# mcgill-cpslab/all-pairs-similarity

Hardware: AMD Instinct MI355X
Metric: scored candidate pairs/sec + achieved HBM GB/s, N=1M d=100k nnz=100, 1/2/4/8 GPU (higher is better)
Workload: dtype u16+f32

## Files before the change

### all-pairs-similarity_amd/csrc/apss_even.hpp

```cpp
#pragma once
#include "apss_kernels.hpp"

namespace apss {

template <int BLOCK, int U, int LONGCAP, bool SHARD, bool SIGNED, bool ACC8, bool MERGE>
__device__ __forceinline__ void probe_even_body(const ProbeArgs &a) {
  constexpr int NW = BLOCK / kWave;
  static_assert(NW == 8 || NW == 16, "8 or 16 waves");
  constexpr int NS = NW - 1;
  constexpr bool SLOT2 = BLOCK <= 512;
  constexpr uint32_t ABITS = ACC8 ? 8u : 16u;
  constexpr bool WIDE = ACC8 && BLOCK > 512;
  constexpr int CH = 16, LPC = CH / 2, GPW = kWave / LPC, WIN = GPW * U;
  constexpr int SLOTS = 2 * WIN < 48 ? 2 * WIN : (WIN > 48 ? WIN : 48);
  static_assert(SLOTS >= WIN, "the register window reads the first WIN slots of a strip");
  constexpr int GS = BLOCK > 512 ? SLOTS / GPW : ((SLOTS / GPW) + 1) & ~1;
  constexpr int SSZ = GPW * GS;
  static_assert(GPW == 8 && SLOTS % GPW == 0, "slot <-> (step, group) by shifts");
  constexpr int kLongLen = kLongLenW;
  constexpr int CBMAX = WIDE ? 131072 : (BLOCK <= 512 && !ACC8 ? 32768 : 65536);
  constexpr int APW = 32 / (int)ABITS;
  constexpr bool LEAN = !SIGNED;
  static_assert(1 + (NW - 1) * 2 * U < (1 << (ACC8 ? 8 : 16)), "the spare words' low accumulators must not wrap within a round");
  __shared__ __attribute__((aligned(16))) uint32_t acc[CBMAX / APW + kWave];
  __shared__ __attribute__((aligned(16))) uint2 strips[3 * NS * SSZ + kWave];
  __shared__ uint2 longs[3 * LONGCAP];
  __shared__ float long_w[3 * LONGCAP];
  __shared__ uint2 facts[4];
  __shared__ unsigned long long stat[4];
  unsigned char *const smem_raw = reinterpret_cast<unsigned char *>(acc);
  uint32_t *const facts_w = reinterpret_cast<uint32_t *>(facts);

  const int tid = threadIdx.x;
  const int wv = __builtin_amdgcn_readfirstlane(tid / kWave), ln = tid % kWave;
  const int cb = a.cb;
  const int F = a.flat_waves;
  const int A = NW - F;
  const int CAP = A * SLOTS;
  const uint32_t A8 = (uint32_t)A * (uint32_t)GPW;
  const float rcpA8 = 1.0f / (float)A8;
  const uint32_t magicA8 = 0xffffffffu / A8 + 1u;
  const int LOGG = a.flat_group_log2, G = 1 << LOGG;
  const uint32_t sub = (uint32_t)ln & (uint32_t)(G - 1);
  const int tile = a.tile0 + blockIdx.x / a.n_chunks;
  const int chunk = blockIdx.x % a.n_chunks;
  static_assert(!MERGE || SHARD, "merged rounds: term shards only");
  const int mlaunch = MERGE ? a.merge_log2 : 0;
  const int c0 = chunk * a.q_chunk;
  const int row_lo = c0 << mlaunch, row_hi = MERGE ? min(a.nq_rows, (c0 + a.q_chunk) << mlaunch) : 0;
  const bool own_tile = mlaunch != 0 && a.q_slot_base >= 0 && (a.q_slot_base + row_lo) / cb <= tile && tile <= (a.q_slot_base + row_hi - 1) / cb;
  const int mlog = own_tile ? 0 : mlaunch;
  const int v0 = row_lo >> mlog;
  const int v1 = own_tile ? row_hi : min(a.nq, c0 + a.q_chunk);
  const int nv = own_tile ? a.nq_rows : a.nq;
  const int qtile = row_lo / cb;
  if (a.tri && tile > qtile) return;
  const int64_t tile_row0 = (int64_t)tile * cb;
  const int unmerged_mark = own_tile ? kUnmergedBit : 0;
  const uint32_t lo = (uint32_t)(ln % LPC);
  const float cxs = a.cx_scale;

  const int64_t qbase = a.q_rowptr[MERGE ? min(v0 << mlog, a.nq_rows) : v0], qend = a.q_rowptr[MERGE ? min(v1 << mlog, a.nq_rows) : v1];
  const int64_t pbase = a.tile_post_base[tile], pend = a.tile_post_base[tile + 1];
  const __amdgpu_buffer_rsrc_t rs_qi =
      __builtin_amdgcn_make_buffer_rsrc((void *)(a.q_idx + qbase), 0, (int)((qend - qbase) * 4), 0x00020000);
  const __amdgpu_buffer_rsrc_t rs_qv =
      __builtin_amdgcn_make_buffer_rsrc((void *)(a.q_val + qbase), 0, (int)((qend - qbase) * 4), 0x00020000);
  const __amdgpu_buffer_rsrc_t rs_tp = __builtin_amdgcn_make_buffer_rsrc(
      (void *)(a.tile_seg + (int64_t)tile * a.seg_stride), 0, (int)(a.seg_stride * 8), 0x00020000);
  const __amdgpu_buffer_rsrc_t rs_po =
      __builtin_amdgcn_make_buffer_rsrc((void *)(a.post_c + pbase), 0, (int)((pend - pbase) * 4), 0x00020000);
  constexpr uint32_t kOob = 0xfffffff0u;
  constexpr uint32_t kStale = 0x80000000u, kSwept = 0x40000000u;
  constexpr uint32_t kRare = 0x80000000u;
  constexpr uint32_t kCountMask = 0xffffu;
  constexpr int kFirstSkippable = BLOCK > 512 || !SHARD ? U - 1 : 0;

  for (int i = tid * 4; i < cb / APW; i += BLOCK * 4) *reinterpret_cast<uint4 *>(acc + i) = make_uint4(0u, 0u, 0u, 0u);
  if (tid < kWave) acc[CBMAX / APW + tid] = 1u;
  if (LEAN) {
    for (int i = tid; i < 3 * NS * SSZ; i += BLOCK) strips[i].x = kStale;
  }
  if (tid < 8) facts_w[tid] = 0;
  unsigned long long my_visits = 0;
  uint32_t my_cands = 0;
  uint32_t n_seen = 0;

  struct RowExt { int qb; int nnz; };
  struct TermW { uint32_t term; float w, qs; bool valid; };
  struct Seg { uint32_t s, len; float w; };
  struct WaveWork {
    uint32_t info;
    uint32_t flags;
    apss_u32x2 pc[U];
    float wq[U];
  };
  const int32_t *const rowptr_lo = reinterpret_cast<const int32_t *>(a.q_rowptr);
  const int qbase_lo = (int)(uint32_t)qbase;
  auto load_R = [&](int v) {
    RowExt r;
    const int row_a = min(v, nv - 1) << mlog, row_b = MERGE ? min(row_a + (1 << mlog), a.nq_rows) : row_a + 1;
    r.qb = rowptr_lo[2 * row_a];
    r.nnz = rowptr_lo[2 * row_b];
    return r;
  };
  auto load_I = [&](const RowExt &r, const int fi, const int v) {
    TermW t;
    const int kterm = ((fi * kWave) >> LOGG) + (ln >> LOGG);
    const int nnz = v < v1 ? r.nnz - r.qb : 0;
    t.valid = kterm < nnz;
    const uint32_t off = t.valid ? (uint32_t)(r.qb - qbase_lo + kterm) * 4u : kOob;
// ... 336 lines not shown
            *reinterpret_cast<unsigned short *>(smem_raw + (w0.pc[u].x & 0xffffu)) = 0;
            *reinterpret_cast<unsigned short *>(smem_raw + (w0.pc[u].y & 0xffffu)) = 0;
          } else {
            acc16w[w0.pc[u].x & 0xffffu] = 0;
            acc16w[w0.pc[u].y & 0xffffu] = 0;
          }
        }
      }
      __syncthreads();
    };
    int r0 = 0;
    for (int v = v0; v < v1; v += 2) {
      round(wfa, wfb, v, r0);
      r0 = r0 == 2 ? 0 : r0 + 1;
      if (v + 1 >= v1) break;
      round(wfb, wfa, v + 1, r0);
      r0 = r0 == 2 ? 0 : r0 + 1;
    }
  }
  __syncthreads();
  if (tid < 3) stat[tid] = 0;
  __syncthreads();
  atomicAdd(&stat[0], my_visits);
  atomicAdd(&stat[1], (unsigned long long)(my_cands - n_seen));
  __syncthreads();
  if (tid == 0) {
    const unsigned long long twice = a.tri && tile < qtile ? 2ull : 1ull;
    atomicAdd(&a.counters[kCtrVisits], stat[0] * twice);
    atomicAdd(&a.counters[kCtrCands], stat[1] * twice);
    atomicAdd(&a.counters[kCtrDevVisits], stat[0]);
  }
}

template <int BLOCK, int U, int LONGCAP, bool SHARD, bool SIGNED, bool ACC8>
__global__ __launch_bounds__(BLOCK, BLOCK <= 512 ? 2 * BLOCK / 256 : BLOCK / 256) void k_probe_even(const ProbeArgs a) {
  probe_even_body<BLOCK, U, LONGCAP, SHARD, SIGNED, ACC8, false>(a);
}

template <int U, bool ACC8>
__global__ __launch_bounds__(512, 4) void k_probe_even_merged(const ProbeArgs a) {
  probe_even_body<512, U, 128, true, false, ACC8, true>(a);
}

}
```

### all-pairs-similarity_amd/csrc/apss_hip.hip

```cpp
#include <hip/hip_runtime.h>

#include <algorithm>
#include <cmath>
#include <cstdio>
#include <cstdlib>
#include <cstring>
#include <new>
#include <string>
#include <vector>

#include "../../include/apss.h"
#include "apss_kernels.hpp"
#include "apss_head.hpp"
#include "apss_even.hpp"
#include "apss_topk.hpp"
#include "apss_window.hpp"

using namespace apss;

namespace {

thread_local std::string g_create_error;

template <class T>
struct DevBuf {
  T *p = nullptr;
  size_t cap = 0;
};

struct DebugCfg {
  bool build_lds = false;
  bool build_atomic = false;
  bool build_stream = false;
  bool build_runs = false;
  int run_range = 0;
  int run_lanes = 0;
  int run_sub = -1;
  bool build_trace = false;
  bool chunk8 = false;
  bool shard_exact = false;
  bool diag = false;
  bool force_general = false;
  bool exact_accum = false;
  bool big_u5 = false;
  int cx_tile = 0;
  int window = 0;
  int chunks = 0;
  int tiles_per_launch = 0;
  bool no_tail = false;
  bool no_acc8 = false;
  int flat_group = -1;
  int pad_lds = 0;
  bool longpf = false;
  bool even_wide = false;
  bool no_even = false;
  int seg_align = 0;
  bool bank_order = false;
  int fold_w = 0;
  bool no_sym = false;
  int mix = 0;
  bool no_chain = false;
  bool no_append = false;
  bool no_bucket = false;
  int bucket_range = 0;
  int res_cap = 0;
  bool head_bf16 = false;
  int merge = -1;
  bool no_merge_prune = false;
  int merge_u = 0;
  int merge_single = 0;
  bool no_fused_ingest = false;
};

DebugCfg parse_debug_env() {
  DebugCfg d;
  const char *e = getenv("APSS_DEBUG");
  if (!e) return d;
  std::string str(e);
  size_t pos = 0;
  while (pos <= str.size()) {
    const size_t end = std::min(str.find(',', pos), str.size());
    const std::string tok = str.substr(pos, end - pos);
    pos = end + 1;
    const size_t eq = tok.find('=');
    const std::string key = tok.substr(0, eq);
    const int val = eq == std::string::npos ? 1 : atoi(tok.c_str() + eq + 1);
    if (key == "build_lds") d.build_lds = val != 0;
    else if (key == "build_atomic") d.build_atomic = val != 0;
    else if (key == "build_stream") d.build_stream = val != 0;
    else if (key == "build_runs") d.build_runs = val != 0;
    else if (key == "run_range") d.run_range = val;
    else if (key == "run_lanes") d.run_lanes = val;
    else if (key == "run_sub") d.run_sub = val;
    else if (key == "build_trace") d.build_trace = val != 0;
    else if (key == "chunk8") d.chunk8 = val != 0;
    else if (key == "shard_exact") d.shard_exact = val != 0;
    else if (key == "diag") d.diag = val != 0;
    else if (key == "force_general") d.force_general = val != 0;
    else if (key == "exact_accum") d.exact_accum = val != 0;
    else if (key == "big_u5") d.big_u5 = val != 0;
    else if (key == "cx_tile") d.cx_tile = val;
    else if (key == "window") d.window = val;
    else if (key == "chunks") d.chunks = val;
    else if (key == "tiles_per_launch") d.tiles_per_launch = val;
    else if (key == "no_tail") d.no_tail = val != 0;
    else if (key == "no_acc8") d.no_acc8 = val != 0;
    else if (key == "no_even") d.no_even = val != 0;
    else if (key == "even_wide") d.even_wide = val != 0;
    else if (key == "longpf") d.longpf = val != 0;
    else if (key == "pad_lds") d.pad_lds = (int)val;
    else if (key == "flat_group") d.flat_group = (int)val;
    else if (key == "seg_align") d.seg_align = val;
    else if (key == "bank_order") d.bank_order = val != 0;
    else if (key == "fold_w") d.fold_w = val;
    else if (key == "mix") d.mix = val;
    else if (key == "no_sym") d.no_sym = val != 0;
    else if (key == "no_chain") d.no_chain = val != 0;
    else if (key == "no_append") d.no_append = val != 0;
    else if (key == "head_bf16") d.head_bf16 = val != 0;
    else if (key == "res_cap") d.res_cap = val;
    else if (key == "no_bucket") d.no_bucket = val != 0;
    else if (key == "bucket_range") d.bucket_range = val;
    else if (key == "merge") d.merge = (int)val;
    else if (key == "merge_u") d.merge_u = (int)val;
    else if (key == "no_merge_prune") d.no_merge_prune = val != 0;
    else if (key == "merge_single") d.merge_single = (int)val;
    else if (key == "no_fused_ingest") d.no_fused_ingest = val != 0;
    else if (key == "relayout_fail") {}
    else if (!key.empty()) fprintf(stderr, "[apss] unknown APSS_DEBUG token '%s' ignored\n", key.c_str());
  }
  return d;
}

}

struct apss_handle {
  apss_config cfg{};
  DebugCfg dbgcfg;
  int dev = 0;
  hipStream_t own_stream = nullptr;
  hipStream_t stream = nullptr;
  hipEvent_t ev0 = nullptr, ev1 = nullptr;
  std::string err;
  bool sharded = false;
  bool nonneg = true;
  bool q_nonneg = true;
  bool no_acc8 = false;
  uint32_t downgrades = 0;
  int64_t store_max_nnz = 0, q_max_nnz = 0;
  float store_max_norm2 = 0.f, q_max_norm2 = 0.f;
  int64_t store_nonempty = 0;
  int64_t last_batch_nonempty = 0;
  int32_t cb = 16384;
  bool stored_rows = false;

  int64_t n_rows = 0, nnz = 0;
  int64_t idx_rows = 0;
  DevBuf<int64_t> rowptr, ext;
  DevBuf<int32_t> idx;
  DevBuf<uint32_t> erow;
// ... 83 lines not shown
    DevBuf<uint32_t> erow;
    int64_t rows = 0, nnz = 0, max_nnz = 0, nonempty = 0, last_nonempty = 0;
  };
  TailView tv, qtv;
  DevBuf<int64_t> tv_cnt, tv_off;
  DevBuf<unsigned int> tv_sum;
  DevBuf<uint16_t> W, q_W;
  bool head_i8 = false;
  float head_s = 0.f;
  DevBuf<unsigned int> head_ovf;
  DevBuf<uint32_t> df;
  DevBuf<unsigned long long> dedup_tab, head_ctr;
  DevBuf<int32_t> uq_q, uq_c;
  DevBuf<float> uq_s;
  int64_t head_nonempty = 0, last_batch_head_nonempty = 0;
  double head_sample_frac = 0.0;
  hipEvent_t ev2 = nullptr, ev3 = nullptr;
  int32_t top_k = 0;
  TopkWork topk;
  apss_topk_info tk{};
  int64_t top_k_window = 0;
  DevBuf<unsigned int> win_df;
  DevBuf<int32_t> win_b;
  DevBuf<int32_t> win_q, win_c;
  DevBuf<float> win_s;
  std::vector<int64_t> win_cuts;
  apss_topk_window_info tw{};
  int64_t win_nonempty = -1, win_head_nonempty = -1;
  bool tile_cut = false, cut_ran = false;
  int64_t cut_uncut = 0, cut_rounds = 0;
  DevBuf<uint32_t> row_pairs;
  apss_topk_tile_cut_info tci{};
  int64_t probe_reruns = 0;
  apss_stats st{};
  size_t bytes_reserved = 0;
};

namespace {

#define HIPCHK(h, expr)                                                                              \
  do {                                                                                               \
    hipError_t e_ = (expr);                                                                          \
    if (e_ != hipSuccess) {                                                                          \
      (h)->err = std::string(#expr) + ": " + hipGetErrorString(e_);                                  \
      return e_ == hipErrorOutOfMemory ? APSS_E_NOMEM : APSS_E_DEVICE;                               \
    }                                                                                                \
  } while (0)

#define APSS_TRY(expr)          \
  do {                          \
    int32_t rc_ = (expr);       \
    if (rc_ != APSS_OK) return rc_; \
  } while (0)

int32_t fail(apss_handle *h, int32_t rc, const std::string &msg) {
  h->err = msg;
  return rc;
}

template <class T>
int32_t ensure(apss_handle *h, DevBuf<T> &b, size_t n, size_t keep = 0, bool exact = false) {
  if (n <= b.cap && b.p) return APSS_OK;
  size_t ncap = exact ? n : std::max(n, b.cap + b.cap / 2);
  ncap = std::max<size_t>(ncap, 64);
  T *np = nullptr;
  HIPCHK(h, hipMalloc((void **)&np, ncap * sizeof(T)));
// ... 1159 lines not shown
  X(1024, 3, false, false, false)      \
  X(1024, 7, false, false, true)       \
  X(1024, 6, false, false, true)       \
  X(1024, 5, false, false, true)       \
  X(1024, 3, false, false, true)
#define APSS_EVEN_MERGE_VARIANTS(X) \
  X(7, false) X(6, false) X(5, false) X(4, false) X(3, false) X(2, false) \
  X(7, true) X(6, true) X(5, true) X(4, true) X(3, true) X(2, true)

bool cx_variant_exists(const CxVariant &v) {
  if (v.even && v.merge) {
#define X(U, A8) \
    if (v.block == 512 && v.u == U && v.shard && !v.sgn && v.acc8 == A8) return v.chunk == 16 && !v.vrows && !v.longpf;
    APSS_EVEN_MERGE_VARIANTS(X)
#undef X
    return false;
  }
  if (v.even) {
#define X(B, U, SH, SG, A8) \
    if (v.block == B && v.u == U && v.shard == SH && v.sgn == SG && v.acc8 == A8) return v.chunk == 16 && !v.vrows && !v.longpf;
    APSS_EVEN_VARIANTS(X)
#undef X
    return false;
  }
#define X(B, U, SH, CH, VR, SG, LP, A8)                                                                                 \
  if (v.block == B && v.u == U && v.shard == SH && v.chunk == CH && v.vrows == VR && v.sgn == SG && v.longpf == LP &&   \
      v.acc8 == A8)                                                                                                     \
    return true;
  APSS_CX_VARIANTS(X)
#undef X
  return false;
}

int32_t launch_cx(apss_handle *h, const CxVariant &v, const ProbeArgs &a) {
  const dim3 grid((unsigned)((int64_t)a.n_tiles * a.n_chunks));
  if (v.even && v.merge) {
#define X(U, A8)                                                                                                           \
    if (v.block == 512 && v.u == U && v.acc8 == A8) {                                                                      \
      hipLaunchKernelGGL((k_probe_even_merged<U, A8>), grid, dim3(512), (size_t)h->dbgcfg.pad_lds, h->stream, a);           \
      HIPCHK(h, hipGetLastError());                                                                                        \
      return APSS_OK;                                                                                                      \
    }
    APSS_EVEN_MERGE_VARIANTS(X)
#undef X
    return fail(h, APSS_E_UNSUPPORTED, "no filter kernel for this combination of options");
  }
  if (v.even) {
#define X(B, U, SH, SG, A8)                                                                                                \
    if (v.block == B && v.u == U && v.shard == SH && v.sgn == SG && v.acc8 == A8) {                                        \
      hipLaunchKernelGGL((k_probe_even<B, U, (B <= 512 ? 128 : 256), SH, SG, A8>), grid, dim3(B),                          \
                         (size_t)h->dbgcfg.pad_lds, h->stream, a);                                                                                 \
      HIPCHK(h, hipGetLastError());                                                                                        \
      return APSS_OK;                                                                                                      \
    }
    APSS_EVEN_VARIANTS(X)
#undef X
    return fail(h, APSS_E_UNSUPPORTED, "no filter kernel for this combination of options");
  }
#define X(B, U, SH, CH, VR, SG, LP, A8)                                                                                    \
  if (v.block == B && v.u == U && v.shard == SH && v.chunk == CH && v.vrows == VR && v.sgn == SG && v.longpf == LP &&      \
      v.acc8 == A8) {                                                                                                      \
    hipLaunchKernelGGL((k_probe_coarse<B, U, (B <= 512 ? 128 : 256), (B <= 512 ? 512 : 1024), SH, CH, VR, SG, LP, A8>), grid, dim3(B), \
                       0, h->stream, a);                                                                                   \
    HIPCHK(h, hipGetLastError());                                                                                          \
    return APSS_OK;                                                                                                        \
  }
  APSS_CX_VARIANTS(X)
#undef X
// ... 575 lines not shown
    if (variant == 'A') APSS_LAUNCH_WAVE(512, 8, 256, 1024);
    else APSS_LAUNCH_WAVE(512, 5, 128, 512);
#undef APSS_LAUNCH_WAVE1
#undef APSS_LAUNCH_WAVE
    HIPCHK(h, hipGetLastError());
    return APSS_OK;
  };

  if (coarse_path && s_max_nnz > vrow_part) APSS_TRY(cut_long_queries(h, s_rowptr, nq, vrow_part, a));
  const int64_t total_tiles = ix.n_tiles;
  int64_t tiles_per_launch = std::max<int64_t>(1, total_tiles);
  if (total_tiles > 0) {
    const double per_tile = (double)s_nnz_end * ((double)idx_nnz / (double)total_tiles / (double)h->cfg.dim) + 1.0;
    tiles_per_launch = (int64_t)std::min<double>((double)total_tiles, std::max(1.0, std::floor(2e11 / per_tile)));
    if (dbg.tiles_per_launch > 0) tiles_per_launch = dbg.tiles_per_launch;
    tiles_per_launch = std::min<int64_t>(tiles_per_launch, std::max<int64_t>(1, 2000000000LL / std::max(1, a.n_chunks)));
  }
  int64_t want_cap = std::min<int64_t>(2 * nq, 1LL << 28);
  if (hybrid_wanted && h->head_sample_frac > 0.0)
    want_cap = std::min<int64_t>(want_cap + (int64_t)(1.5 * h->head_sample_frac * (double)nq * (double)h->idx_rows), 1LL << 30);
  else if (hybrid_wanted && h->sharded)
    want_cap = std::min<int64_t>(want_cap + 6 * nq, 1LL << 30);
  if (h->res_q.cap < (size_t)want_cap) {
    const size_t cap0 = (size_t)(dbg.res_cap > 0 ? dbg.res_cap : std::max<int64_t>(1 << 20, want_cap));
    APSS_TRY(ensure(h, h->res_q, cap0, 0, true));
    APSS_TRY(ensure(h, h->res_c, cap0, 0, true));
    APSS_TRY(ensure(h, h->res_s, cap0, 0, true));
  }
  if (hybrid) APSS_TRY(ensure(h, h->head_ctr, 4));
  constexpr int64_t kChainMaxQueries = 65536;
  const bool chain = coarse_path && !h->sharded && !hybrid && !tri && nq <= kChainMaxQueries && !dbg.no_chain;
  const int64_t chain_tail_pairs = chain ? nq * tail_n : 0;
  if (chain) APSS_TRY(ensure(h, h->chain_ctr, kCtrCount));
  for (int attempt = 0; attempt < 3; ++attempt) {
    if (chain) {
      const size_t fin_cap = h->res_q.cap + (size_t)(nq * std::max<int64_t>(tail_n, kTailMaxRows));
      APSS_TRY(ensure(h, h->fin_q, fin_cap));
      APSS_TRY(ensure(h, h->fin_c, fin_cap));
      APSS_TRY(ensure(h, h->fin_s, fin_cap));
    }
    if (a.merge_log2 > 0) {
      APSS_TRY(ensure(h, h->res2_q, h->res_q.cap, 0, true));
      APSS_TRY(ensure(h, h->res2_c, h->res_q.cap, 0, true));
      APSS_TRY(ensure(h, h->res2_s, h->res_q.cap, 0, true));
    }
    a.dbg = nullptr;
    a.res_q = h->res_q.p;
    a.res_c = h->res_c.p;
    a.res_s = h->res_s.p;
    a.res_cap = h->res_q.cap;
    HIPCHK(h, hipMemsetAsync(h->counters.p, 0, kCtrCount * sizeof(unsigned long long), h->stream));
    if (gen_cut) HIPCHK(h, hipMemsetAsync(h->row_pairs.p, 0, (size_t)nq * sizeof(uint32_t), h->stream));
    HIPCHK(h, hipEventRecord(h->ev0, h->stream));
    int64_t n_launches = 0, thin_launches = 0;
    {
      auto tf = [](bool b) { return b ? "true" : "false"; };
      char *nm = h->st.probe_kernel;
      const size_t cap = sizeof(h->st.probe_kernel);
      if (coarse_path && cxv.even)
        if (cxv.merge) snprintf(nm, cap, "k_probe_even_merged<%d, %s>", cxv.u, tf(cxv.acc8));
        else snprintf(nm, cap, "k_probe_even<%d, %d, %d, %s, %s, %s>", cxv.block, cxv.u, cxv.block <= 512 ? 128 : 256, tf(cxv.shard), tf(cxv.sgn), tf(cxv.acc8));
      else if (coarse_path)
        snprintf(nm, cap, "k_probe_coarse<%d, %d, %d, %d, %s, %d, %s, %s, %s, %s>", cxv.block, cxv.u, cxv.block <= 512 ? 128 : 256,
                 cxv.block <= 512 ? 512 : 1024, tf(cxv.shard), cxv.chunk, tf(cxv.vrows), tf(cxv.sgn), tf(cxv.longpf), tf(cxv.acc8));
      else if (wave_path)
        snprintf(nm, cap, "k_probe_wave<%d, %d, %d, %d, %s, %s>", wave_block, wave_u, wave_longcap, wave_survcap, tf(h->sharded), tf(dbg.diag));
      else if (gen_cut)
        snprintf(nm, cap, "k_probe<%d, %d, %s, true>", mode, gen_block(mode, h->ex.cb), tf(gen_fx));
      else
        snprintf(nm, cap, "k_probe<%d, %d, %s>", mode, gen_block(mode, h->ex.cb), tf(gen_fx));
    }
    for (int64_t t0 = 0; t0 < total_tiles; t0 += tiles_per_launch, ++n_launches) {
      a.tile0 = (int32_t)t0;
      a.n_tiles = (int32_t)std::min<int64_t>(tiles_per_launch, total_tiles - t0);
      if (coarse_path) {
        APSS_TRY(launch_cx(h, cxv, a));
        thin_launches += cxv.even ? 1 : 0;
      } else if (wave_path && dbg.diag) {
        APSS_TRY(ensure(h, h->dbg, 8));
        HIPCHK(h, hipMemsetAsync(h->dbg.p, 0, 8 * sizeof(unsigned long long), h->stream));
        a.dbg = h->dbg.p;
        APSS_TRY(launch_wave(true));
        unsigned long long d[8];
        HIPCHK(h, hipMemcpyAsync(d, h->dbg.p, sizeof(d), hipMemcpyDeviceToHost, h->stream));
        HIPCHK(h, hipStreamSynchronize(h->stream));
        unsigned long long tot = 0;
        for (int k = 0; k < 7; ++k) tot += d[k];
        fprintf(stderr, "[apss diag] stage+flatten %.1f%% | atomics %.1f%% | longs/rest %.1f%% | barrier G %.1f%% | survivors %.1f%% | "
                        "re-zero %.1f%% | barrier U %.1f%% | cycles/round/wave %.0f\n",
                100.0 * d[0] / tot, 100.0 * d[1] / tot, 100.0 * d[2] / tot, 100.0 * d[3] / tot, 100.0 * d[4] / tot,
                100.0 * d[5] / tot, 100.0 * d[6] / tot, (double)tot / ((double)a.n_tiles * a.nq * (wave_block / kWave)));
      } else if (wave_path) {
        APSS_TRY(launch_wave(false));
      } else if (gen_cut) {
        const bool b512 = gen_block(2, h->ex.cb) == 512;
        if (gen_fx && b512) APSS_TRY((launch_probe<2, true, 512, true>(h, a, lds)));
        else if (gen_fx) APSS_TRY((launch_probe<2, true, kProbeBlock, true>(h, a, lds)));
        else if (b512) APSS_TRY((launch_probe<2, false, 512, true>(h, a, lds)));
        else APSS_TRY((launch_probe<2, false, kProbeBlock, true>(h, a, lds)));
      } else if (gen_fx) {
        if (mode == 0) APSS_TRY((launch_probe<0, true>(h, a, lds)));
        else if (mode == 1) APSS_TRY((launch_probe<1, true>(h, a, lds)));
        else if (gen_block(2, h->ex.cb) == 512) APSS_TRY((launch_probe<2, true, 512>(h, a, lds)));
        else APSS_TRY((launch_probe<2, true>(h, a, lds)));
      } else {
        if (mode == 0) APSS_TRY((launch_probe<0, false>(h, a, lds)));
        else if (mode == 1) APSS_TRY((launch_probe<1, false>(h, a, lds)));
        else if (gen_block(2, h->ex.cb) == 512) APSS_TRY((launch_probe<2, false, 512>(h, a, lds)));
// ... 23 lines not shown
        sp.cap = a.res_cap;
        sp.q_rowptr = s_rowptr;
        sp.q_idx = s_idx;
        sp.q_val = s_val;
        sp.q_sub = q_sub;
        sp.c_rowptr = h->head_k ? h->tv.rowptr.p : h->rowptr.p;
        sp.c_idx = h->head_k ? h->tv.idx.p : h->idx.p;
        sp.c_val = h->head_k ? h->tv.val.p : h->val.p;
        sp.c_sub = h->sub.p;
        sp.theta = (float)theta;
        sp.out_q = h->res2_q.p;
        sp.out_c = h->res2_c.p;
        sp.out_s = h->res2_s.p;
        sp.counter = h->counters.p + kCtrResults;
        sp.over = h->counters.p + kCtrOver;
        const int64_t grid_pairs = std::min<int64_t>((int64_t)a.res_cap, nq / 4 + 4096);
        hipLaunchKernelGGL(k_shard_prune, dim3((unsigned)std::min<int64_t>(2048, ceil_div(grid_pairs, kPrunePairs * 4))), dim3(kPruneBlock), 0, h->stream, sp);
        HIPCHK(h, hipGetLastError());
        std::swap(h->res_q, h->res2_q);
        std::swap(h->res_c, h->res2_c);
        std::swap(h->res_s, h->res2_s);
        a.res_q = h->res_q.p;
        a.res_c = h->res_c.p;
        a.res_s = h->res_s.p;
      }
    }
    if (tri) {
      HIPCHK(h, hipMemcpyAsync(h->counters.p + kCtrSnap, h->counters.p + kCtrResults, sizeof(unsigned long long), hipMemcpyDeviceToDevice, h->stream));
      hipLaunchKernelGGL(k_mirror_survivors, dim3(1024), dim3(256), 0, h->stream, a.res_q, a.res_c, a.res_s,
                         (const unsigned long long *)(h->counters.p + kCtrSnap), (uint64_t)a.res_cap, (int32_t)a.cb, h->counters.p + kCtrResults);
      HIPCHK(h, hipGetLastError());
    }
    HIPCHK(h, hipEventRecord(h->ev1, h->stream));
    unsigned long long cc_stack[kCtrCount] = {0, 0, 0, 0, 0, 0, 0, 0}, c_stack[kCtrCount];
    unsigned long long *cc = h->pin ? reinterpret_cast<unsigned long long *>(h->pin + kPinBytes + 64) : cc_stack;
    unsigned long long *c = h->pin ? reinterpret_cast<unsigned long long *>(h->pin + kPinBytes + 128) : c_stack;
    for (int k = 0; k < kCtrCount; ++k) cc[k] = 0;
    if (chain) {
      HIPCHK(h, hipMemsetAsync(h->chain_ctr.p, 0, kCtrCount * sizeof(unsigned long long), h->stream));
      RescoreArgs r{};
      r.n_pairs = (int64_t)a.res_cap;
      r.n_pairs_dev = h->counters.p + kCtrResults;
      r.q_row = h->res_q.p;
      r.c_slot = h->res_c.p;
      r.q_rowptr = q_rowptr;
      r.q_idx = q_idx;
      r.q_val = q_val;
      r.c_rowptr = h->rowptr.p;
      r.c_idx = h->idx.p;
      r.c_val = h->val.p;
      r.theta = (float)theta;
      r.out_q = h->fin_q.p;
      r.out_c = h->fin_c.p;
      r.out_s = h->fin_s.p;
      r.out_count = h->chain_ctr.p + kCtrResults;
      const int64_t grid_pairs = std::min<int64_t>((int64_t)a.res_cap, 64 * nq + 4096);
      hipLaunchKernelGGL(k_rescore, dim3((unsigned)std::max<int64_t>(1, ceil_div(grid_pairs, (int64_t)kRescorePairs * kRescoreTrips))), dim3(kRescoreBlock), 0, h->stream, r);
      if (tail_n > 0) {
        TailArgs t{};
        t.nq = nq;
        t.n_tail = tail_n;
        t.q_rowptr = q_rowptr;
        t.q_idx = q_idx;
        t.q_val = q_val;
        t.q_ext = q_ext;
        t.c_rowptr = h->rowptr.p;
        t.c_idx = h->idx.p;
        t.c_val = h->val.p;
        t.c_ext = h->ext.p;
// ... 528 lines not shown
    if (ensure(h, h->idx, (size_t)cfg->capacity_nnz, 0, true) != APSS_OK ||
        ensure(h, h->erow, (size_t)cfg->capacity_nnz, 0, true) != APSS_OK ||
        ensure(h, h->val, (size_t)cfg->capacity_nnz, 0, true) != APSS_OK ||
        (h->use_coarse ? ensure(h, h->cx.post_c, (size_t)cfg->capacity_nnz * 2 + 64, 0, true)
                       : ensure(h, h->ex.post, (size_t)cfg->capacity_nnz + (size_t)cfg->capacity_nnz / 2 + 64, 0, true)) != APSS_OK) {
      g_create_error = h->err;
      apss_destroy(h);
      return APSS_E_NOMEM;
    }
  }
  *out = h;
  return APSS_OK;
}

void apss_destroy(apss_handle *h) {
  if (!h) return;
  (void)hipSetDevice(h->dev);
  if (h->own_stream) (void)hipStreamSynchronize(h->own_stream);
  release(h->rowptr); release(h->ext); release(h->idx); release(h->erow); release(h->val); release(h->sub);
  for (apss_handle::IndexSet *s : {&h->ex, &h->cx}) { release(s->seg); release(s->post); release(s->post_c); release(s->base); release(s->total); release(s->maxlen); release(s->chunkw); release(s->scan_part); }
  release(h->tile_min); release(h->tile_min_c); release(h->fin_q); release(h->fin_c); release(h->fin_s);
  release(h->q_rowptr); release(h->q_ext); release(h->q_idx); release(h->q_val); release(h->q_sub);
  release(h->s_keep); release(h->s_cnt); release(h->s_rowdst); release(h->s_nnzdst); release(h->scan_tmp);
  release(h->in_rowptr); release(h->in_ext); release(h->in_idx); release(h->s_inv); release(h->s_sub); release(h->in_val); release(h->in_val64); release(h->vq_first); release(h->vrow_q); release(h->vrow_ptr); release(h->vrow_np); release(h->vrow_first);
  release(h->res_q); release(h->res_c); release(h->res_s); release(h->res2_q); release(h->res2_c); release(h->res2_s); release(h->q_prenorm); release(h->counters); release(h->flagword); release(h->dbg);
  release(h->head_pos); release(h->W);
  for (apss_handle::TailView *v : {&h->tv, &h->qtv}) { release(v->rowptr); release(v->idx); release(v->val); release(v->erow); }
  release(h->tv_cnt); release(h->tv_off); release(h->tv_sum); release(h->q_W); release(h->df); release(h->dedup_tab);
  release(h->head_ctr); release(h->uq_q); release(h->uq_c); release(h->uq_s); release(h->pack); release(h->chain_ctr); release(h->app_seg); release(h->app_post); release(h->bk_cnt); release(h->bk_base); release(h->bk_idx); release(h->bk_erow); release(h->bk_val); release(h->run_cut); release(h->run_ent); release(h->ing_cut);
  topk_release(h->topk);
  release(h->win_df); release(h->win_b); release(h->win_q); release(h->win_c); release(h->win_s);
  release(h->row_pairs);
  if (h->pin) (void)hipHostFree(h->pin);
  if (h->ev0) (void)hipEventDestroy(h->ev0);
  if (h->ev1) (void)hipEventDestroy(h->ev1);
  if (h->ev2) (void)hipEventDestroy(h->ev2);
  if (h->ev3) (void)hipEventDestroy(h->ev3);
  if (h->own_stream) (void)hipStreamDestroy(h->own_stream);
  delete h;
}

const char *apss_last_error(const apss_handle *h) { return h ? h->err.c_str() : g_create_error.c_str(); }

int32_t apss_set_stream(apss_handle *h, void *hip_stream, int32_t use_own) {
  APSS_TRY(enter(h));
  HIPCHK(h, hipStreamSynchronize(h->stream));
  h->stream = use_own ? h->own_stream : (hipStream_t)hip_stream;
  return APSS_OK;
}

int32_t apss_insert(apss_handle *h, int64_t n, const int64_t *rowptr, const int32_t *indices, const double *values,
                    const int64_t *ext_ids) {
  APSS_TRY(enter(h));
  APSS_TRY(validate_host_csr(h, n, rowptr, indices, values, ext_ids));
  if (n == 0) return APSS_OK;
  APSS_TRY(upload(h, n, rowptr, indices, values, ext_ids));
  int64_t first = 0;
  return insert_dev_impl(h, n, rowptr[n], h->up_rowptr, h->up_idx, h->in_val.p, h->up_ext, &first);
}

int32_t apss_query(apss_handle *h, int64_t n, const int64_t *rowptr, const int32_t *indices, const double *values,
                   const int64_t *ext_ids, int64_t *n_results) {
  APSS_TRY(enter(h));
  APSS_TRY(validate_host_csr(h, n, rowptr, indices, values, ext_ids));
  APSS_TRY(upload(h, n, rowptr, indices, values, ext_ids));
  return query_dev_impl(h, n, n ? rowptr[n] : 0, h->up_rowptr, h->up_idx, h->in_val.p, h->up_ext, n_results);
// ... 379 lines not shown
```

### all-pairs-similarity_amd/csrc/apss_kernels.hpp

```cpp
#pragma once
#include <hip/hip_fp16.h>
#include <hip/hip_runtime.h>
#include <stdint.h>

#include "apss_topk_key.hpp"

namespace apss {

constexpr int kWave = 64;
constexpr int kGroup = 16;
constexpr int kItemCap = 2048;
constexpr int kLongCap = 256;
constexpr int kLongLen = 64;
constexpr int kSurvCap = 1024;
constexpr int kProbeBlock = 1024;

struct alignas(8) Posting {
  uint32_t slot;
  float w;
};

template <typename T>
__device__ __forceinline__ T uniform_load(const T *p) {
  return *reinterpret_cast<const __attribute__((address_space(4))) T *>(reinterpret_cast<uintptr_t>(p));
}

constexpr int kUnmergedBit = 0x40000000;
enum Counter { kCtrResults = 0, kCtrVisits = 1, kCtrCands = 2, kCtrFlags = 3, kCtrDevVisits = 4, kCtrSnap = 5, kCtrPre = 6, kCtrOver = 7, kCtrCount = 8 };

__device__ __forceinline__ uint64_t wave_append(bool pred, unsigned long long *counter) {
  const unsigned long long mask = __ballot(pred);
  if (mask == 0) return ~0ull;
  const int lane = __lane_id();
  const int leader = __ffsll((long long)mask) - 1;
  unsigned long long base = 0;
  if (lane == leader) base = atomicAdd(counter, (unsigned long long)__popcll(mask));
  base = __shfl(base, leader);
  const unsigned long long below = mask & ((1ull << lane) - 1ull);
  return pred ? base + (unsigned long long)__popcll(below) : ~0ull;
}


struct IngestArgs {
  int64_t n;
  int64_t nnz;
  const int64_t *rowptr;
  const int32_t *idx;
  const float *val;
  int32_t dim, term_lo, term_hi;
  uint32_t flags;
  float theta, index_threshold;
  const int32_t *head_pos;
  int64_t *row_keep;
  int64_t *row_cnt;
  float *row_inv;
  float *row_sub;
  unsigned int *flags_out;
};

template <int G>
__global__ void k_ingest_count(IngestArgs a) {
// ... 919 lines not shown
  const int64_t *q_rowptr;
  const int32_t *q_idx;
  const float *q_val;
  const int64_t *q_ext;
  const float *q_scale;
  int64_t q_nnz_end;
  int32_t nq;
  int32_t q_chunk;
  int32_t n_chunks;
  int32_t flat_waves;
  int32_t flat_group_log2;
  int32_t merge_log2;
  int32_t nq_rows;
  int32_t tri;
  int64_t q_slot_base;
  float theta;
  float fx_scale;
  uint32_t theta_fx;
  int32_t theta_fxi;
  const uint32_t *post_c;
  const int32_t *vq_first;
  const int64_t *vrow_ptr;
  const int32_t *vrow_q;
  float cx_scale;
  float cx_theta;
  int32_t *res_q;
  int32_t *res_c;
  float *res_s;
  uint64_t res_cap;
  unsigned long long *counters;
  unsigned long long *dbg;
  uint32_t *row_pairs;
  int32_t cut_k;
};

struct ProbeLds {
  float *acc;
  uint2 *items;
  uint2 *longs;
  float *long_w;
  float *wq;
  uint32_t *surv;
  uint32_t *bitmap;
  uint32_t *ctr;
};

__host__ __device__ inline size_t probe_lds_bytes(int cb, int block, int mode) {
  size_t b = (size_t)cb * 4 + (size_t)kItemCap * 8 + (size_t)kLongCap * 8 + (size_t)kLongCap * 4 +
             (size_t)block * 4 + (size_t)kSurvCap * 4 + 64;
  if (mode == 2) b += (size_t)((cb + 31) / 32 + 3) / 4 * 16;
  return (b + 15) / 16 * 16;
}

__device__ __forceinline__ void probe_hist_add(uint32_t *hist, bool match, uint32_t dig) {
  const unsigned long long m = __ballot(match);
  if (m == 0ull) return;
  const int leader = __ffsll((long long)m) - 1;
  const uint32_t first = (uint32_t)__shfl((int)dig, leader);
  if (__all(!match || dig == first)) {
    if ((int)(threadIdx.x & 63) == leader) atomicAdd(&hist[first], (uint32_t)__popcll(m));
  } else if (match) {
    atomicAdd(&hist[dig], 1u);
  }
}

template <int MODE, int BLOCK, bool FX, bool CUT = false>
// ... 1648 lines not shown
```

Baseline: 1022 billion.

## Run the even probe kernel persistently over a host-built work list

The even-filter probe now launches one workgroup per resident slot and has each workgroup pull (tile, query range) items from a device work list through an atomic counter. The final cells of each launch are split into finer pieces so the tail balances across CUs. The host builds the list once, caches it by shape, and uploads it through pinned memory. Kernel arguments are also read through the constant address space and scalar loads. The intent is to cut tail imbalance and per-block launch overhead, at the cost of an atomic and a barrier per item and a host-side list build whenever the shape changes.

```diff
diff --git a/all-pairs-similarity_amd/csrc/apss_even.hpp b/all-pairs-similarity_amd/csrc/apss_even.hpp
--- a/all-pairs-similarity_amd/csrc/apss_even.hpp
+++ b/all-pairs-similarity_amd/csrc/apss_even.hpp
@@ -3,8 +3,10 @@
 
 namespace apss {
 
+using ProbeArgsK = const __attribute__((address_space(4))) ProbeArgs;
+
 template <int BLOCK, int U, int LONGCAP, bool SHARD, bool SIGNED, bool ACC8, bool MERGE>
-__device__ __forceinline__ void probe_even_body(const ProbeArgs &a) {
+__device__ __forceinline__ void probe_even_item(ProbeArgsK &a, const int tile, const int v0, const int v1, const bool own_tile, const bool first) {
   constexpr int NW = BLOCK / kWave;
   static_assert(NW == 8 || NW == 16, "8 or 16 waves");
   constexpr int NS = NW - 1;
@@ -31,7 +33,8 @@
   unsigned char *const smem_raw = reinterpret_cast<unsigned char *>(acc);
   uint32_t *const facts_w = reinterpret_cast<uint32_t *>(facts);
 
-  const int tid = threadIdx.x;
+  int tid = threadIdx.x;
+  asm volatile("" : "+v"(tid));
   const int wv = __builtin_amdgcn_readfirstlane(tid / kWave), ln = tid % kWave;
   const int cb = a.cb;
   const int F = a.flat_waves;
@@ -42,26 +45,18 @@
   const uint32_t magicA8 = 0xffffffffu / A8 + 1u;
   const int LOGG = a.flat_group_log2, G = 1 << LOGG;
   const uint32_t sub = (uint32_t)ln & (uint32_t)(G - 1);
-  const int tile = a.tile0 + blockIdx.x / a.n_chunks;
-  const int chunk = blockIdx.x % a.n_chunks;
   static_assert(!MERGE || SHARD, "merged rounds: term shards only");
   const int mlaunch = MERGE ? a.merge_log2 : 0;
-  const int c0 = chunk * a.q_chunk;
-  const int row_lo = c0 << mlaunch, row_hi = MERGE ? min(a.nq_rows, (c0 + a.q_chunk) << mlaunch) : 0;
-  const bool own_tile = mlaunch != 0 && a.q_slot_base >= 0 && (a.q_slot_base + row_lo) / cb <= tile && tile <= (a.q_slot_base + row_hi - 1) / cb;
   const int mlog = own_tile ? 0 : mlaunch;
-  const int v0 = row_lo >> mlog;
-  const int v1 = own_tile ? row_hi : min(a.nq, c0 + a.q_chunk);
   const int nv = own_tile ? a.nq_rows : a.nq;
-  const int qtile = row_lo / cb;
-  if (a.tri && tile > qtile) return;
+  const int qtile = (v0 << mlog) / cb;
   const int64_t tile_row0 = (int64_t)tile * cb;
   const int unmerged_mark = own_tile ? kUnmergedBit : 0;
   const uint32_t lo = (uint32_t)(ln % LPC);
   const float cxs = a.cx_scale;
 
-  const int64_t qbase = a.q_rowptr[MERGE ? min(v0 << mlog, a.nq_rows) : v0], qend = a.q_rowptr[MERGE ? min(v1 << mlog, a.nq_rows) : v1];
-  const int64_t pbase = a.tile_post_base[tile], pend = a.tile_post_base[tile + 1];
+  const int64_t qbase = uniform_load(a.q_rowptr + (MERGE ? min(v0 << mlog, a.nq_rows) : v0)), qend = uniform_load(a.q_rowptr + (MERGE ? min(v1 << mlog, a.nq_rows) : v1));
+  const int64_t pbase = uniform_load(a.tile_post_base + tile), pend = uniform_load(a.tile_post_base + tile + 1);
   const __amdgpu_buffer_rsrc_t rs_qi =
       __builtin_amdgcn_make_buffer_rsrc((void *)(a.q_idx + qbase), 0, (int)((qend - qbase) * 4), 0x00020000);
   const __amdgpu_buffer_rsrc_t rs_qv =
@@ -76,7 +71,8 @@
   constexpr uint32_t kCountMask = 0xffffu;
   constexpr int kFirstSkippable = BLOCK > 512 || !SHARD ? U - 1 : 0;
 
-  for (int i = tid * 4; i < cb / APW; i += BLOCK * 4) *reinterpret_cast<uint4 *>(acc + i) = make_uint4(0u, 0u, 0u, 0u);
+  if (first)
+    for (int i = tid * 4; i < cb / APW; i += BLOCK * 4) *reinterpret_cast<uint4 *>(acc + i) = make_uint4(0u, 0u, 0u, 0u);
   if (tid < kWave) acc[CBMAX / APW + tid] = 1u;
   if (LEAN) {
     for (int i = tid; i < 3 * NS * SSZ; i += BLOCK) strips[i].x = kStale;
@@ -479,6 +475,48 @@
   }
 }
 
+template <int BLOCK, int U, int LONGCAP, bool SHARD, bool SIGNED, bool ACC8, bool MERGE>
+__device__ __forceinline__ void probe_even_body(const ProbeArgs &a) {
+  int g_tile = 0, g_v0 = 0, g_v1 = 0;
+  if (!a.items) {
+    const int cb = a.cb, mlaunch = MERGE ? a.merge_log2 : 0;
+    const int tile = a.tile0 + blockIdx.x / a.n_chunks;
+    const int c0 = (blockIdx.x % a.n_chunks) * a.q_chunk;
+    const int row_lo = c0 << mlaunch, row_hi = MERGE ? min(a.nq_rows, (c0 + a.q_chunk) << mlaunch) : 0;
+    const bool own_tile = mlaunch != 0 && a.q_slot_base >= 0 && (a.q_slot_base + row_lo) / cb <= tile && tile <= (a.q_slot_base + row_hi - 1) / cb;
+    if (a.tri && tile > row_lo / cb) return;
+    g_tile = tile | (own_tile ? kUnmergedBit : 0);
+    g_v0 = own_tile ? row_lo : c0;
+    g_v1 = own_tile ? row_hi : min(a.nq, c0 + a.q_chunk);
+    asm volatile("" : "+s"(g_tile), "+s"(g_v0), "+s"(g_v1));
+  }
+  __shared__ int next_item;
+  for (bool first = true;; first = false) {
+    int tile, v0, v1;
+    bool own_tile;
+    if (a.items) {
+      if (threadIdx.x == 0) next_item = (int)atomicAdd(a.work_ctr, 1ull);
+      __syncthreads();
+      const int idx = __builtin_amdgcn_readfirstlane(next_item);
+      if (idx >= a.n_items) return;
+      const ProbeItem *const it = a.items + idx;
+      tile = uniform_load(&it->tile);
+      v0 = uniform_load(&it->v0);
+      v1 = uniform_load(&it->v1);
+      own_tile = uniform_load(&it->own) != 0;
+    } else {
+      if (!first) return;
+      tile = g_tile & ~kUnmergedBit;
+      v0 = g_v0;
+      v1 = g_v1;
+      own_tile = (g_tile & kUnmergedBit) != 0;
+    }
+    ProbeArgsK *ak = reinterpret_cast<ProbeArgsK *>(reinterpret_cast<uintptr_t>(__builtin_amdgcn_kernarg_segment_ptr()));
+    asm volatile("" : "+s"(ak));
+    probe_even_item<BLOCK, U, LONGCAP, SHARD, SIGNED, ACC8, MERGE>(*ak, tile, v0, v1, own_tile, first);
+  }
+}
+
 template <int BLOCK, int U, int LONGCAP, bool SHARD, bool SIGNED, bool ACC8>
 __global__ __launch_bounds__(BLOCK, BLOCK <= 512 ? 2 * BLOCK / 256 : BLOCK / 256) void k_probe_even(const ProbeArgs a) {
   probe_even_body<BLOCK, U, LONGCAP, SHARD, SIGNED, ACC8, false>(a);
diff --git a/all-pairs-similarity_amd/csrc/apss_hip.hip b/all-pairs-similarity_amd/csrc/apss_hip.hip
--- a/all-pairs-similarity_amd/csrc/apss_hip.hip
+++ b/all-pairs-similarity_amd/csrc/apss_hip.hip
@@ -5,6 +5,7 @@
 #include <cstdio>
 #include <cstdlib>
 #include <cstring>
+#include <map>
 #include <new>
 #include <string>
 #include <vector>
@@ -70,6 +71,9 @@
   int merge_u = 0;
   int merge_single = 0;
   bool no_fused_ingest = false;
+  bool no_persist = false;
+  int persist_wgs = 0;
+  int persist_fine = 0;
 };
 
 DebugCfg parse_debug_env() {
@@ -126,6 +130,9 @@
     else if (key == "no_merge_prune") d.no_merge_prune = val != 0;
     else if (key == "merge_single") d.merge_single = (int)val;
     else if (key == "no_fused_ingest") d.no_fused_ingest = val != 0;
+    else if (key == "no_persist") d.no_persist = val != 0;
+    else if (key == "persist_wgs") d.persist_wgs = val;
+    else if (key == "persist_fine") d.persist_fine = val;
     else if (key == "relayout_fail") {}
     else if (!key.empty()) fprintf(stderr, "[apss] unknown APSS_DEBUG token '%s' ignored\n", key.c_str());
   }
@@ -275,6 +282,14 @@
   DevBuf<uint32_t> row_pairs;
   apss_topk_tile_cut_info tci{};
   int64_t probe_reruns = 0;
+  std::vector<apss::WorkListKey> wl_keys;
+  std::vector<int64_t> wl_off, wl_fine;
+  apss::ProbeItem *wl_pin = nullptr;
+  size_t wl_pin_cap = 0;
+  DevBuf<apss::ProbeItem> wl_dev;
+  hipEvent_t wl_ev = nullptr;
+  std::map<const void *, int> wl_per_cu;
+  int n_cus = 0;
   apss_stats st{};
   size_t bytes_reserved = 0;
 };
@@ -1500,8 +1515,38 @@
   return false;
 }
 
-int32_t launch_cx(apss_handle *h, const CxVariant &v, const ProbeArgs &a) {
-  const dim3 grid((unsigned)((int64_t)a.n_tiles * a.n_chunks));
+const void *even_kernel(const CxVariant &v) {
+  if (v.even && v.merge) {
+#define X(U, A8) \
+    if (v.block == 512 && v.u == U && v.acc8 == A8) return reinterpret_cast<const void *>(&k_probe_even_merged<U, A8>);
+    APSS_EVEN_MERGE_VARIANTS(X)
+#undef X
+  } else if (v.even) {
+#define X(B, U, SH, SG, A8) \
+    if (v.block == B && v.u == U && v.shard == SH && v.sgn == SG && v.acc8 == A8) \
+      return reinterpret_cast<const void *>(&k_probe_even<B, U, (B <= 512 ? 128 : 256), SH, SG, A8>);
+    APSS_EVEN_VARIANTS(X)
+#undef X
+  }
+  return nullptr;
+}
+
+int32_t even_resident_slots(apss_handle *h, const CxVariant &v, int *slots) {
+  const void *kern = even_kernel(v);
+  if (!kern) return fail(h, APSS_E_UNSUPPORTED, "no filter kernel for this combination of options");
+  if (h->n_cus == 0) HIPCHK(h, hipDeviceGetAttribute(&h->n_cus, hipDeviceAttributeMultiprocessorCount, h->dev));
+  auto it = h->wl_per_cu.find(kern);
+  if (it == h->wl_per_cu.end()) {
+    int per_cu = 0;
+    HIPCHK(h, hipOccupancyMaxActiveBlocksPerMultiprocessor(&per_cu, kern, v.block, (size_t)h->dbgcfg.pad_lds));
+    it = h->wl_per_cu.emplace(kern, std::max(per_cu, 1)).first;
+  }
+  *slots = it->second * h->n_cus;
+  return APSS_OK;
+}
+
+int32_t launch_cx(apss_handle *h, const CxVariant &v, const ProbeArgs &a, int64_t persist_wgs = 0) {
+  const dim3 grid((unsigned)(persist_wgs > 0 ? persist_wgs : (int64_t)a.n_tiles * a.n_chunks));
   if (v.even && v.merge) {
 #define X(U, A8)                                                                                                           \
     if (v.block == 512 && v.u == U && v.acc8 == A8) {                                                                      \
@@ -2143,6 +2188,59 @@
   const bool chain = coarse_path && !h->sharded && !hybrid && !tri && nq <= kChainMaxQueries && !dbg.no_chain;
   const int64_t chain_tail_pairs = chain ? nq * tail_n : 0;
   if (chain) APSS_TRY(ensure(h, h->chain_ctr, kCtrCount));
+  constexpr int kPersistFine = 128;
+  constexpr int64_t kPersistMaxCells = 1LL << 22;
+  int persist_slots = 0;
+  const bool persist = coarse_path && cxv.even && !dbg.no_persist && total_tiles > 0 && total_tiles * (int64_t)a.n_chunks <= kPersistMaxCells;
+  if (persist) {
+    APSS_TRY(even_resident_slots(h, cxv, &persist_slots));
+    int fine = 1;
+    while (2 * fine <= (dbg.persist_fine > 0 ? dbg.persist_fine : kPersistFine)) fine *= 2;
+    std::vector<apss::WorkListKey> keys;
+    for (int64_t t0 = 0; t0 < total_tiles; t0 += tiles_per_launch) {
+      apss::WorkListKey k;
+      k.q_slot_base = a.merge_log2 > 0 ? q_slot_base : -1;
+      k.nq = a.nq;
+      k.nq_rows = a.nq_rows;
+      k.q_chunk = a.q_chunk;
+      k.n_chunks = a.n_chunks;
+      k.cb = a.cb;
+      k.tri = a.tri;
+      k.merge_log2 = a.merge_log2;
+      k.tile0 = (int32_t)t0;
+      k.n_tiles = (int32_t)std::min<int64_t>(tiles_per_launch, total_tiles - t0);
+      k.fine = fine;
+      k.slots = dbg.persist_wgs > 0 ? dbg.persist_wgs : persist_slots;
+      keys.push_back(k);
+    }
+    if (!(keys == h->wl_keys) || !h->wl_dev.p) {
+      std::vector<apss::ProbeItem> items;
+      h->wl_keys.clear();
+      h->wl_off.assign(1, 0);
+      h->wl_fine.clear();
+      for (const apss::WorkListKey &k : keys) {
+        h->wl_fine.push_back(apss::build_work_list(k, items));
+        h->wl_off.push_back((int64_t)items.size());
+      }
+      if (!h->wl_ev) HIPCHK(h, hipEventCreateWithFlags(&h->wl_ev, hipEventDisableTiming));
+      else HIPCHK(h, hipEventSynchronize(h->wl_ev));
+      if (items.size() > h->wl_pin_cap) {
+        if (h->wl_pin) (void)hipHostFree(h->wl_pin);
+        h->wl_pin = nullptr;
+        h->wl_pin_cap = 0;
+        const size_t cap = std::max<size_t>(items.size() + items.size() / 2, 4096);
+        HIPCHK(h, hipHostMalloc((void **)&h->wl_pin, cap * sizeof(apss::ProbeItem), hipHostMallocDefault));
+        h->wl_pin_cap = cap;
+      }
+      APSS_TRY(ensure(h, h->wl_dev, std::max<size_t>(items.size(), 1)));
+      if (!items.empty()) {
+        std::memcpy(h->wl_pin, items.data(), items.size() * sizeof(apss::ProbeItem));
+        HIPCHK(h, hipMemcpyAsync(h->wl_dev.p, h->wl_pin, items.size() * sizeof(apss::ProbeItem), hipMemcpyHostToDevice, h->stream));
+      }
+      HIPCHK(h, hipEventRecord(h->wl_ev, h->stream));
+      h->wl_keys = keys;
+    }
+  }
   for (int attempt = 0; attempt < 3; ++attempt) {
     if (chain) {
       const size_t fin_cap = h->res_q.cap + (size_t)(nq * std::max<int64_t>(tail_n, kTailMaxRows));
@@ -2184,7 +2282,18 @@
     for (int64_t t0 = 0; t0 < total_tiles; t0 += tiles_per_launch, ++n_launches) {
       a.tile0 = (int32_t)t0;
       a.n_tiles = (int32_t)std::min<int64_t>(tiles_per_launch, total_tiles - t0);
-      if (coarse_path) {
+      if (coarse_path && persist) {
+        if (n_launches > 0) HIPCHK(h, hipMemsetAsync(h->counters.p + kCtrWork, 0, sizeof(unsigned long long), h->stream));
+        const int64_t n_items = h->wl_off[n_launches + 1] - h->wl_off[n_launches];
+        a.items = h->wl_dev.p + h->wl_off[n_launches];
+        a.n_items = (int32_t)n_items;
+        a.work_ctr = h->counters.p + kCtrWork;
+        const int64_t wgs = std::min<int64_t>(n_items, dbg.persist_wgs > 0 ? dbg.persist_wgs : persist_slots);
+        if (dbg.diag)
+          fprintf(stderr, "[apss diag] persist: items %lld fine %lld workgroups %lld\n", (long long)n_items, (long long)h->wl_fine[n_launches], (long long)wgs);
+        if (wgs > 0) APSS_TRY(launch_cx(h, cxv, a, wgs));
+        thin_launches += 1;
+      } else if (coarse_path) {
         APSS_TRY(launch_cx(h, cxv, a));
         thin_launches += cxv.even ? 1 : 0;
       } else if (wave_path && dbg.diag) {
@@ -2274,9 +2383,9 @@
       HIPCHK(h, hipGetLastError());
     }
     HIPCHK(h, hipEventRecord(h->ev1, h->stream));
-    unsigned long long cc_stack[kCtrCount] = {0, 0, 0, 0, 0, 0, 0, 0}, c_stack[kCtrCount];
-    unsigned long long *cc = h->pin ? reinterpret_cast<unsigned long long *>(h->pin + kPinBytes + 64) : cc_stack;
-    unsigned long long *c = h->pin ? reinterpret_cast<unsigned long long *>(h->pin + kPinBytes + 128) : c_stack;
+    unsigned long long cc_stack[kCtrCount] = {}, c_stack[kCtrCount];
+    unsigned long long *cc = h->pin ? reinterpret_cast<unsigned long long *>(h->pin + kPinBytes + 128) : cc_stack;
+    unsigned long long *c = h->pin ? reinterpret_cast<unsigned long long *>(h->pin + kPinBytes + 256) : c_stack;
     for (int k = 0; k < kCtrCount; ++k) cc[k] = 0;
     if (chain) {
       HIPCHK(h, hipMemsetAsync(h->chain_ctr.p, 0, kCtrCount * sizeof(unsigned long long), h->stream));
@@ -2871,6 +2980,9 @@
   release(h->win_df); release(h->win_b); release(h->win_q); release(h->win_c); release(h->win_s);
   release(h->row_pairs);
   if (h->pin) (void)hipHostFree(h->pin);
+  release(h->wl_dev);
+  if (h->wl_pin) (void)hipHostFree(h->wl_pin);
+  if (h->wl_ev) (void)hipEventDestroy(h->wl_ev);
   if (h->ev0) (void)hipEventDestroy(h->ev0);
   if (h->ev1) (void)hipEventDestroy(h->ev1);
   if (h->ev2) (void)hipEventDestroy(h->ev2);
diff --git a/all-pairs-similarity_amd/csrc/apss_kernels.hpp b/all-pairs-similarity_amd/csrc/apss_kernels.hpp
--- a/all-pairs-similarity_amd/csrc/apss_kernels.hpp
+++ b/all-pairs-similarity_amd/csrc/apss_kernels.hpp
@@ -4,6 +4,7 @@
 #include <stdint.h>
 
 #include "apss_topk_key.hpp"
+#include "apss_worklist.hpp"
 
 namespace apss {
 
@@ -26,7 +27,7 @@
 }
 
 constexpr int kUnmergedBit = 0x40000000;
-enum Counter { kCtrResults = 0, kCtrVisits = 1, kCtrCands = 2, kCtrFlags = 3, kCtrDevVisits = 4, kCtrSnap = 5, kCtrPre = 6, kCtrOver = 7, kCtrCount = 8 };
+enum Counter { kCtrResults = 0, kCtrVisits = 1, kCtrCands = 2, kCtrFlags = 3, kCtrDevVisits = 4, kCtrSnap = 5, kCtrPre = 6, kCtrOver = 7, kCtrWork = 8, kCtrCount = 9 };
 
 __device__ __forceinline__ uint64_t wave_append(bool pred, unsigned long long *counter) {
   const unsigned long long mask = __ballot(pred);
@@ -1012,6 +1013,9 @@
   unsigned long long *dbg;
   uint32_t *row_pairs;
   int32_t cut_k;
+  int32_t n_items;
+  const ProbeItem *items;
+  unsigned long long *work_ctr;
 };
 
 struct ProbeLds {
diff --git a/all-pairs-similarity_amd/csrc/apss_worklist.hpp b/all-pairs-similarity_amd/csrc/apss_worklist.hpp
--- /dev/null
+++ b/all-pairs-similarity_amd/csrc/apss_worklist.hpp
@@ -0,0 +1,63 @@
+#pragma once
+#include <algorithm>
+#include <cstdint>
+#include <vector>
+
+namespace apss {
+
+struct alignas(16) ProbeItem {
+  int32_t tile;
+  int32_t v0, v1;
+  int32_t own;
+};
+
+struct WorkListKey {
+  int64_t q_slot_base = -1;
+  int32_t nq = 0;
+  int32_t nq_rows = 0;
+  int32_t q_chunk = 0;
+  int32_t n_chunks = 0;
+  int32_t cb = 0;
+  int32_t tri = 0;
+  int32_t merge_log2 = 0;
+  int32_t tile0 = 0, n_tiles = 0;
+  int32_t fine = 0;
+  int32_t slots = 0;
+  bool operator==(const WorkListKey &o) const {
+    return q_slot_base == o.q_slot_base && nq == o.nq && nq_rows == o.nq_rows && q_chunk == o.q_chunk && n_chunks == o.n_chunks &&
+           cb == o.cb && tri == o.tri && merge_log2 == o.merge_log2 && tile0 == o.tile0 && n_tiles == o.n_tiles && fine == o.fine &&
+           slots == o.slots;
+  }
+};
+
+inline bool work_cell(const WorkListKey &k, int32_t tile, int32_t chunk, ProbeItem &it) {
+  const int m = k.merge_log2;
+  const int64_t c0 = (int64_t)chunk * k.q_chunk;
+  const int64_t row_lo = c0 << m, row_hi = std::min<int64_t>(k.nq_rows, (c0 + k.q_chunk) << m);
+  if (k.tri && tile > row_lo / k.cb) return false;
+  const bool own = m != 0 && k.q_slot_base >= 0 && (k.q_slot_base + row_lo) / k.cb <= tile && tile <= (k.q_slot_base + row_hi - 1) / k.cb;
+  it.tile = tile;
+  it.own = own ? 1 : 0;
+  it.v0 = (int32_t)(own ? row_lo : c0);
+  it.v1 = (int32_t)(own ? row_hi : std::min<int64_t>(k.nq, c0 + k.q_chunk));
+  return it.v1 > it.v0;
+}
+
+inline int64_t build_work_list(const WorkListKey &k, std::vector<ProbeItem> &out) {
+  const size_t first = out.size();
+  ProbeItem it;
+  for (int32_t tile = k.tile0; tile < k.tile0 + k.n_tiles; ++tile)
+    for (int32_t chunk = 0; chunk < k.n_chunks; ++chunk)
+      if (work_cell(k, tile, chunk, it)) out.push_back(it);
+  if (k.fine <= 0 || k.fine >= k.q_chunk || k.slots <= 0) return 0;
+  const size_t n = out.size() - first;
+  const size_t n_cut = std::min<size_t>(n, 2 * (size_t)k.slots);
+  std::vector<ProbeItem> cut(out.end() - (std::ptrdiff_t)n_cut, out.end());
+  out.resize(out.size() - n_cut);
+  int64_t n_fine = 0;
+  for (const ProbeItem &c : cut)
+    for (int32_t v = c.v0; v < c.v1; v += k.fine, ++n_fine) out.push_back(ProbeItem{c.tile, v, std::min(c.v1, v + k.fine), c.own});
+  return n_fine;
+}
+
+}
diff --git a/all-pairs-similarity_amd/host/worklist_selftest.cpp b/all-pairs-similarity_amd/host/worklist_selftest.cpp
--- /dev/null
+++ b/all-pairs-similarity_amd/host/worklist_selftest.cpp
@@ -0,0 +1,137 @@
+#include <cstdio>
+#include <cstdlib>
+#include <map>
+#include <tuple>
+#include <vector>
+
+#include "../csrc/apss_worklist.hpp"
+
+using apss::ProbeItem;
+using apss::WorkListKey;
+
+namespace {
+
+int failures = 0;
+#define CHECK(cond, ...)                       \
+  do {                                         \
+    if (!(cond)) {                             \
+      ++failures;                              \
+      std::fprintf(stderr, "FAIL %s: ", name); \
+      std::fprintf(stderr, __VA_ARGS__);       \
+      std::fprintf(stderr, "\n");              \
+    }                                          \
+  } while (0)
+
+struct Cell {
+  int tile, v0, v1;
+  bool own;
+};
+
+bool grid_cell(const WorkListKey &k, int64_t b, Cell &c) {
+  const int mlaunch = k.merge_log2;
+  const int tile = k.tile0 + (int)(b / k.n_chunks);
+  const int c0 = (int)(b % k.n_chunks) * k.q_chunk;
+  const int row_lo = c0 << mlaunch;
+  const int row_hi = mlaunch ? std::min(k.nq_rows, (c0 + k.q_chunk) << mlaunch) : 0;
+  const bool own = mlaunch != 0 && k.q_slot_base >= 0 && (k.q_slot_base + row_lo) / k.cb <= tile && tile <= (k.q_slot_base + row_hi - 1) / k.cb;
+  if (k.tri && tile > row_lo / k.cb) return false;
+  c.tile = tile;
+  c.own = own;
+  c.v0 = own ? row_lo : c0;
+  c.v1 = own ? row_hi : std::min(k.nq, c0 + k.q_chunk);
+  return true;
+}
+
+void check_shape(const char *name, const WorkListKey &k) {
+  std::vector<ProbeItem> items;
+  const int64_t n_fine = apss::build_work_list(k, items);
+  std::map<std::tuple<int, int, int>, int> todo;
+  std::vector<Cell> cells;
+  for (int64_t b = 0; b < (int64_t)k.n_tiles * k.n_chunks; ++b) {
+    Cell c;
+    if (!grid_cell(k, b, c)) continue;
+    cells.push_back(c);
+    for (int v = c.v0; v < c.v1; ++v) todo[std::make_tuple(c.tile, (int)c.own, v)] += 1;
+  }
+  size_t rounds = todo.size();
+  for (const ProbeItem &it : items) {
+    CHECK(it.v1 > it.v0, "empty item tile %d [%d, %d)", it.tile, it.v0, it.v1);
+    for (int v = it.v0; v < it.v1; ++v) {
+      auto f = todo.find(std::make_tuple(it.tile, it.own, v));
+      CHECK(f != todo.end() && f->second == 1, "round %d of tile %d (own %d) is not the grid's, or covered twice", v, it.tile, it.own);
+      if (f != todo.end()) f->second -= 1;
+    }
+    if (k.tri) {
+      const int mlog = it.own ? 0 : k.merge_log2;
+      const int64_t lo = (int64_t)it.v0 << mlog, hi = std::min<int64_t>(k.nq_rows, (int64_t)it.v1 << mlog);
+      CHECK(lo / k.cb == (hi - 1) / k.cb, "item [%d, %d) straddles a query tile", it.v0, it.v1);
+      CHECK(it.tile <= lo / k.cb, "item of tile %d above the diagonal (query tile %lld)", it.tile, (long long)(lo / k.cb));
+    }
+  }
+  for (const auto &kv : todo) CHECK(kv.second == 0, "round %d of tile %d left uncovered", std::get<2>(kv.first), std::get<0>(kv.first));
+  const size_t n_whole = items.size() - (size_t)n_fine;
+  CHECK(n_fine >= 0 && (size_t)n_fine <= items.size(), "pieces %lld of %zu items", (long long)n_fine, items.size());
+  for (size_t i = 0; i < n_whole && i < cells.size(); ++i)
+    CHECK(items[i].tile == cells[i].tile && items[i].v0 == cells[i].v0 && items[i].v1 == cells[i].v1 && (items[i].own != 0) == cells[i].own,
+          "item %zu is not cell %zu of the grid", i, i);
+  for (size_t i = n_whole; i < items.size(); ++i) {
+    CHECK(items[i].v1 - items[i].v0 <= k.fine, "piece %zu is %d rounds long (fine %d)", i, items[i].v1 - items[i].v0, k.fine);
+    if (i > n_whole) CHECK(items[i].tile >= items[i - 1].tile, "piece %zu leaves the tile-major order", i);
+  }
+  if (n_fine > 0) {
+    const size_t want_cut = std::min<size_t>(cells.size(), 2 * (size_t)k.slots);
+    CHECK(n_whole == cells.size() - want_cut, "%zu whole items, want %zu cells - %zu cut", n_whole, cells.size(), want_cut);
+  } else {
+    CHECK(items.size() == cells.size(), "%zu items for %zu cells", items.size(), cells.size());
+  }
+  std::printf("%-28s cells %6zu rounds %9zu items %6zu pieces %6lld\n", name, cells.size(), rounds, items.size(), (long long)n_fine);
+}
+
+WorkListKey shape(int nq_rows, int merge_log2, int want_chunks, int cb, int tri, int64_t q_slot_base, int tile0, int n_tiles, int fine, int slots) {
+  WorkListKey k;
+  const int M = 1 << merge_log2;
+  int q_chunk = std::max(1, (nq_rows + want_chunks - 1) / want_chunks);
+  if (tri) {
+    int qc = 1;
+    while (qc < q_chunk) qc <<= 1;
+    q_chunk = qc;
+  }
+  const int qc_rows = (q_chunk + M - 1) / M * M;
+  k.q_chunk = qc_rows / M;
+  k.n_chunks = (nq_rows + qc_rows - 1) / qc_rows;
+  k.nq = (nq_rows + M - 1) / M;
+  k.nq_rows = nq_rows;
+  k.merge_log2 = merge_log2;
+  k.cb = cb;
+  k.tri = tri;
+  k.q_slot_base = q_slot_base;
+  k.tile0 = tile0;
+  k.n_tiles = n_tiles;
+  k.fine = fine;
+  k.slots = slots;
+  return k;
+}
+
+}
+
+int main() {
+  check_shape("c3 symmetric", shape(1000000, 0, 1024, 32768, 1, 0, 0, 31, 256, 512));
+  check_shape("c3 symmetric fine 128", shape(1000000, 0, 1024, 32768, 1, 0, 0, 31, 128, 512));
+  check_shape("c3 two-directional", shape(1000000, 0, 1024, 32768, 0, 0, 0, 31, 256, 512));
+  check_shape("small symmetric", shape(4100, 0, 32, 1024, 1, 0, 0, 5, 16, 4));
+  check_shape("small symmetric all cut", shape(4100, 0, 32, 1024, 1, 0, 0, 5, 8, 4096));
+  check_shape("outside batch fine 1", shape(777, 0, 13, 512, 0, -1, 2, 3, 1, 3));
+  check_shape("outside batch fine 2", shape(778, 0, 7, 512, 0, -1, 0, 4, 2, 1));
+  check_shape("nothing cut", shape(300, 0, 64, 1024, 0, -1, 0, 2, 256, 512));
+  check_shape("one item", shape(5, 0, 1, 1024, 0, -1, 0, 1, 256, 512));
+  check_shape("merged whole store", shape(6001, 1, 24, 1024, 0, 0, 0, 6, 32, 2));
+  check_shape("merged appended", shape(2049, 1, 16, 1024, 0, 1500, 0, 4, 16, 3));
+  check_shape("merged outside", shape(2049, 2, 16, 1024, 0, -1, 0, 4, 16, 3));
+  check_shape("merged symmetric", shape(5000, 1, 20, 1024, 1, 0, 0, 5, 64, 2));
+  if (failures) {
+    std::fprintf(stderr, "%d check(s) failed\n", failures);
+    return 1;
+  }
+  std::printf("worklist selftest ok\n");
+  return 0;
+}
```

New measurement: 1061 billion (median of 6 runs). +3.8%, better.
